# SowpatiLab/ribbit

Hardware: AMD Instinct MI355X
Metric: Gbases/s scanned (m=2..100) (higher is better)
Workload: dtype u32 bit planes

## Files before the change

### ribbit_amd/csrc/kernels.hip

```cpp
#include <hip/hip_runtime.h>

#include <algorithm>
#include <climits>
#include <type_traits>

#include "kernels.h"

namespace rb {

__device__ __forceinline__ uint32_t funnel(uint32_t hi, uint32_t lo, uint32_t sh) {
    return __builtin_amdgcn_alignbit(hi, lo, sh);
}

template <unsigned TT>
__device__ __forceinline__ uint32_t bitop3(uint32_t a, uint32_t b, uint32_t c) {
    return __builtin_amdgcn_bitop3_b32(a, b, c, TT);
}

__global__ __launch_bounds__(256) void pack_kernel(const uint8_t *__restrict__ ascii, int64_t length,
                                                   uint32_t *__restrict__ hi, uint32_t *__restrict__ lo,
                                                   uint32_t *__restrict__ brk, int64_t total_words,
                                                   uint32_t *__restrict__ zero_words, int n_zero) {
    const int64_t t = (int64_t)blockIdx.x * blockDim.x + threadIdx.x;
    if (blockIdx.x == 0)
// ... 103 lines not shown
    int cnt = 0;
#pragma unroll
    for (int k = 0; k < WORDS_PER_LANE; k++) cnt += __popc(Sv[k]) + __popc(Ev[k]);
    const int incl = wave_inclusive_scan(cnt);
    const int total = __builtin_amdgcn_readlane(incl, 63);
    if (staged + total > EV_STAGE) sink_flush(sink, stage, staged, lane);
    const bool direct = total > EV_STAGE;
    uint32_t idx = (uint32_t)(incl - cnt);
    uint64_t *gdst = nullptr;
    if (direct) {
        uint32_t base = 0;
        if (lane == 0) base = atomicAdd(&sink.counters[sink.shard * EV_COUNTER_STRIDE], (uint32_t)total);
        idx += (uint32_t)__builtin_amdgcn_readfirstlane((int)base);
        gdst = sink.events + (size_t)sink.shard * sink.region_cap;
    } else {
        idx += (uint32_t)staged;
    }
#pragma unroll
    for (int k = 0; k < WORDS_PER_LANE; k++) {
        uint32_t both = Sv[k] | Ev[k];
        while (both) {
            const uint32_t b = (uint32_t)__builtin_ctz(both);
            both &= both - 1u;
            const uint32_t pos = ((word0 + (uint32_t)k) << 5) + b;
            const uint32_t kind = ((Sv[k] >> b) & 1u) ? (uint32_t)EV_START : end_kind(k, b, pos);
            const uint64_t e = ev_pack(pos, mlen, kind);
            if (direct) { if (idx < sink.region_cap) gdst[idx] = e; }
            else stage[idx] = e;
            idx++;
        }
    }
    if (!direct) staged += total;
    __builtin_amdgcn_wave_barrier();
}

constexpr int K = WORDS_PER_LANE;

#ifndef RB_COOP_MAX_LANES
#define RB_COOP_MAX_LANES 16
#endif
constexpr int COOP_SRC = 16;
struct CoopScratch { uint32_t w[COOP_SRC][20]; };

__device__ __forceinline__ void stage_events_coop(const uint32_t (&S)[WORDS_PER_LANE], const uint32_t (&E)[WORDS_PER_LANE], uint32_t word0, uint32_t mlen,
                                                  uint32_t brk_at, const uint32_t *s_brk, uint32_t length, CoopScratch &sc, const EventSink &sink,
                                                  volatile uint64_t *stage, int &staged, int lane) {
    uint32_t Sv[WORDS_PER_LANE], Ev[WORDS_PER_LANE];
#pragma unroll
    for (int k = 0; k < WORDS_PER_LANE; k++) {
        Sv[k] = S[k]; Ev[k] = E[k];
        asm volatile("" : "+v"(Sv[k]), "+v"(Ev[k]));
    }
    int cnt = 0;
#pragma unroll
    for (int k = 0; k < WORDS_PER_LANE; k++) cnt += __popc(Sv[k] | Ev[k]);
    const int incl = wave_inclusive_scan(cnt);
    const int total = __builtin_amdgcn_readlane(incl, 63);
    if (staged + total > EV_STAGE) sink_flush(sink, stage, staged, lane);
    const bool direct = total > EV_STAGE;
    uint32_t first = (uint32_t)(incl - cnt);
    uint64_t *gdst = nullptr;
    if (direct) {
        uint32_t base = 0;
        if (lane == 0) base = atomicAdd(&sink.counters[sink.shard * EV_COUNTER_STRIDE], (uint32_t)total);
        first += (uint32_t)__builtin_amdgcn_readfirstlane((int)base);
        gdst = sink.events + (size_t)sink.shard * sink.region_cap;
    } else {
        first += (uint32_t)staged;
    }
    unsigned long long todo = __ballot(cnt != 0);
    const int r = lane >> 2, j = lane & 3;
    do {
        const int rank = (int)__builtin_amdgcn_mbcnt_hi((uint32_t)(todo >> 32), __builtin_amdgcn_mbcnt_lo((uint32_t)todo, 0u));
        const bool mine = ((todo >> lane) & 1ull) != 0ull && rank < COOP_SRC;
        if (mine) {
            uint32_t *row = sc.w[rank];
#pragma unroll
            for (int k = 0; k < WORDS_PER_LANE; k++) { row[k] = Sv[k]; row[WORDS_PER_LANE + k] = Ev[k]; }
            row[16] = word0; row[17] = mlen; row[18] = brk_at; row[19] = first;
        }
        const unsigned long long handled = __ballot(mine);
        const int nsrc = __popcll(handled);
        todo &= ~handled;
        __builtin_amdgcn_wave_barrier();
        uint32_t s0 = 0, s1 = 0, e0 = 0, e1 = 0;
        if (r < nsrc) { s0 = sc.w[r][2 * j]; s1 = sc.w[r][2 * j + 1]; e0 = sc.w[r][WORDS_PER_LANE + 2 * j]; e1 = sc.w[r][WORDS_PER_LANE + 2 * j + 1]; }
        const int c = __popc(s0 | e0) + __popc(s1 | e1);
        const int q0 = __builtin_amdgcn_update_dpp(0, c, 0x00, 0xf, 0xf, true);
        const int q1 = __builtin_amdgcn_update_dpp(0, c, 0x55, 0xf, 0xf, true);
        const int q2 = __builtin_amdgcn_update_dpp(0, c, 0xaa, 0xf, 0xf, true);
        if (c != 0) {
            const uint32_t w0 = sc.w[r][16], ml = sc.w[r][17], bb = sc.w[r][18];
            uint32_t idx = sc.w[r][19] + (uint32_t)((j > 0 ? q0 : 0) + (j > 1 ? q1 : 0) + (j > 2 ? q2 : 0));
            auto expand = [&](uint32_t sw, uint32_t ew, uint32_t k) {
                uint32_t both = sw | ew;
                while (both) {
                    const uint32_t b = (uint32_t)__builtin_ctz(both);
                    both &= both - 1u;
                    const uint32_t pos = ((w0 + k) << 5) + b;
                    uint32_t kind = (uint32_t)EV_START;
                    if (!((sw >> b) & 1u))
                        kind = pos >= length ? (uint32_t)EV_END_EOS : (((s_brk[bb + k] >> b) & 1u) ? (uint32_t)EV_END_N : (uint32_t)EV_END_ZERO);
                    const uint64_t e = ev_pack(pos, ml, kind);
                    if (direct) { if (idx < sink.region_cap) gdst[idx] = e; }
                    else stage[idx] = e;
                    idx++;
                }
            };
            expand(s0, e0, 2u * (uint32_t)j);
            expand(s1, e1, 2u * (uint32_t)j + 1u);
        }
        __builtin_amdgcn_wave_barrier();
    } while (RB_COOP_MAX_LANES > COOP_SRC && todo != 0ull);
    if (!direct) staged += total;
}
__device__ __forceinline__ void group_filter(const uint32_t (&PASS)[K + 2], const uint32_t (&EVAL)[K + 2], int tj, uint32_t (&SV)[K + 1],
                                             uint32_t (&DR)[K]) {
    uint32_t J[K + 2], W[K + 2];
#pragma unroll
    for (int j = K + 1; j >= 1; j--) J[j] = PASS[j] | funnel(PASS[j], PASS[j - 1], 31);
    J[0] = PASS[0] | (PASS[0] << 1);
#pragma unroll
    for (int j = K + 1; j >= 1; j--) J[j] = J[j] | funnel(J[j], J[j - 1], 30);
    J[0] = J[0] | (J[0] << 2);
#pragma unroll
    for (int j = K + 1; j >= 1; j--) J[j] = J[j] | funnel(J[j], J[j - 1], 28);
    J[0] = J[0] | (J[0] << 4);
#pragma unroll
    for (int j = 0; j < K + 1; j++) J[j] = J[j] & funnel(J[j + 1], J[j], 1);
    J[K + 1] = J[K + 1] & (J[K + 1] >> 1);
#pragma unroll
    for (int j = 0; j < K + 1; j++) J[j] = J[j] & funnel(J[j + 1], J[j], 2);
    J[K + 1] = J[K + 1] & (J[K + 1] >> 2);
#pragma unroll
    for (int j = 0; j < K + 1; j++) J[j] = J[j] & funnel(J[j + 1], J[j], 4);
    J[K + 1] = J[K + 1] & (J[K + 1] >> 4);
#pragma unroll
    for (int j = 0; j < K + 2; j++) J[j] |= PASS[j];
#pragma unroll
    for (int j = 0; j < K + 2; j++) W[j] = J[j];
    {
        int span = 1;
#pragma unroll
        for (int step = 0; step < 4; step++) {
            const int sh = min(span, tj - span);
            if (sh > 0) {
#pragma unroll
                for (int j = 0; j < K + 1; j++) W[j] = W[j] & funnel(W[j + 1], W[j], (uint32_t)sh);
                W[K + 1] = W[K + 1] & (W[K + 1] >> sh);
                span += sh;
            }
        }
        span = 1;
#pragma unroll
        for (int step = 0; step < 4; step++) {
            const int sh = min(span, tj - span);
            if (sh > 0) {
#pragma unroll
                for (int j = K + 1; j >= 1; j--) W[j] = W[j] | funnel(W[j], W[j - 1], (uint32_t)(32 - sh));
                W[0] = W[0] | (W[0] << sh);
                span += sh;
            }
        }
    }
    auto special_ends = [&](int j) {
        const uint32_t jprev = j > 0 ? funnel(J[j], J[j - 1], 31) : (J[0] << 1);
        const uint32_t ev8 = j < K + 1 ? funnel(EVAL[j + 1], EVAL[j], 8) : (EVAL[K + 1] >> 8);
        const uint32_t g = ~J[j] & jprev & ~(EVAL[j] & ev8);
        return j == 0 ? 0u : (j == K + 1 ? (g & 0x0000ffffu) : g);
    };
    uint32_t special = 0;
#pragma unroll
    for (int j = 1; j < K + 2; j++) special |= special_ends(j);
    if (__ballot(special != 0) != 0ull) {
        uint32_t G[K + 2], JL[K + 2];
#pragma unroll
        for (int j = 0; j < K + 2; j++) { JL[j] = J[j]; G[j] = special_ends(j); }
#pragma unroll
        for (int j = 0; j < K + 1; j++) G[j] = funnel(G[j + 1], G[j], 1) & J[j];
        G[K + 1] = (G[K + 1] >> 1) & J[K + 1];
#pragma unroll
        for (int sh = 1; sh <= 8; sh <<= 1) {
#pragma unroll
            for (int j = 0; j < K + 1; j++) G[j] |= funnel(G[j + 1], G[j], (uint32_t)sh) & JL[j];
            G[K + 1] |= (G[K + 1] >> sh) & JL[K + 1];
#pragma unroll
            for (int j = 0; j < K + 1; j++) JL[j] = JL[j] & funnel(JL[j + 1], JL[j], (uint32_t)sh);
            JL[K + 1] = JL[K + 1] & (JL[K + 1] >> sh);
        }
#pragma unroll
        for (int j = 0; j < K + 1; j++) W[j] |= G[j];
    }
#pragma unroll
    for (int j = 0; j < K + 1; j++) SV[j] = W[j];
#pragma unroll
    for (int k = 0; k < K; k++) {
        const uint32_t jprev = funnel(J[k + 1], J[k], 31);
        const uint32_t svprev = funnel(W[k + 1], W[k], 31);
        DR[k] = ~J[k + 1] & jprev & ~svprev;
    }
}

constexpr int LDS_EXTRA = 40;

template <bool UNIFORM>
__device__ __forceinline__ uint32_t perfect_edges(const uint32_t (&Z)[K + 2], uint32_t t3, uint32_t t4, uint32_t t5,
                                                  uint32_t back, uint32_t (&SQ)[K], uint32_t (&EQ)[K]) {
    uint32_t D[K + 2];
#pragma unroll
    for (int j = 0; j < K + 1; j++) D[j] = Z[j] | funnel(Z[j + 1], Z[j], 1);
    D[K + 1] = Z[K + 1] | (Z[K + 1] >> 1);
#pragma unroll
    for (int j = 0; j < K + 1; j++) D[j] = D[j] | funnel(D[j + 1], D[j], 2);
    D[K + 1] = D[K + 1] | (D[K + 1] >> 2);
#pragma unroll
    for (int j = 0; j < K + 1; j++) D[j] = D[j] | funnel(D[j + 1], D[j], t3);
    D[K + 1] = D[K + 1] | (D[K + 1] >> t3);
#pragma unroll
    for (int j = 0; j < K + 1; j++) D[j] = D[j] | funnel(D[j + 1], D[j], t4);
    if (!UNIFORM || t5) {
        D[K + 1] = D[K + 1] | (D[K + 1] >> t4);
#pragma unroll
        for (int j = 0; j < K + 1; j++) D[j] = D[j] | funnel(D[j + 1], D[j], t5);
    }
    uint32_t any = 0;
#pragma unroll
    for (int k = 0; k < K; k++) {
        const int j = k + 1;
        const uint32_t prev_z = funnel(Z[j], Z[j - 1], 31);
        const uint32_t d_back = funnel(D[j], D[j - 1], back);
        SQ[k] = prev_z & ~D[j];
        EQ[k] = Z[j] & ~d_back;
        any = bitop3<0xFE>(SQ[k], EQ[k], any);
    }
    return any;
}

constexpr int CAND_CAP = 64;
#ifndef RB_CAND_DIRECT
#define RB_CAND_DIRECT 32
#endif
constexpr int CAND_DIRECT = RB_CAND_DIRECT;
struct CandQueue {
    uint32_t z[K + 2][CAND_CAP];
    uint32_t tag[CAND_CAP];
};

#ifndef RB_PERFECT_WAVES
#define RB_PERFECT_WAVES 4
#endif
__global__ __launch_bounds__(256) __attribute__((amdgpu_waves_per_eu(RB_PERFECT_WAVES, RB_PERFECT_WAVES))) void scan_perfect_kernel(DevicePlanes pl, PerfectLaunch pp, int motifs_per_block,
                                                           uint64_t *__restrict__ events,
                                                           uint32_t *__restrict__ counters) {
    __shared__ uint32_t s_hi[TILE_WORDS + LDS_EXTRA];
    __shared__ uint32_t s_lo[TILE_WORDS + LDS_EXTRA];
    __shared__ uint32_t s_brk[TILE_WORDS + 8];
    __shared__ uint64_t s_stage[4][EV_STAGE];
    __shared__ CandQueue s_cand[4];
    __shared__ CoopScratch s_coop[4];

    const int lane = threadIdx.x & 63;
    const int wave = __builtin_amdgcn_readfirstlane((int)(threadIdx.x >> 6));
    const int64_t tile_base = (int64_t)blockIdx.x * TILE_WORDS;

    const int bm_lo = pp.m_lo + (int)blockIdx.y * motifs_per_block;
    const int bm_hi = min(pp.m_hi, bm_lo + motifs_per_block - 1);
    const int q_hi = bm_hi >> 5;

    const int n_ext = TILE_WORDS + 4 + q_hi;
    for (int i = threadIdx.x; i < n_ext; i += 256) {
        s_hi[i] = pl.hi[tile_base - 1 + i];
        s_lo[i] = pl.lo[tile_base - 1 + i];
    }
    for (int i = threadIdx.x; i < TILE_WORDS + 2; i += 256) s_brk[i] = pl.brk[tile_base - 1 + i];
    __syncthreads();

    const int wm_lo = bm_lo + wave;
    const int wm_hi = bm_hi;
    if (wm_lo > wm_hi) return;

    const int lb = lane * K;
    uint32_t H[K + 2], Lo[K + 2], Bk[K + 2];
#pragma unroll
    for (int j = 0; j < K + 2; j++) { H[j] = s_hi[lb + j]; Lo[j] = s_lo[lb + j]; Bk[j] = s_brk[lb + j]; }

    uint32_t Hq[K + 3], Lq[K + 3];
    int cur_q = -1;
    const uint32_t length = (uint32_t)pl.length;
    const uint32_t word0 = (uint32_t)(tile_base + lb);

    EventSink sink;
    sink.events = events;
    sink.counters = counters;
    sink.region_cap = pp.ev_cap / EV_SHARDS;
    sink.shard = (blockIdx.x * 4u + (uint32_t)wave + blockIdx.y) % EV_SHARDS;
    volatile uint64_t *stage = s_stage[wave];
    int staged = 0;

    CandQueue &cq = s_cand[wave];
    int queued = 0;
    auto flush_candidates = [&]() {
        if (queued == 0) return;
        const bool live = lane < queued;
        const uint32_t tag = live ? cq.tag[lane] : 0u;
        const uint32_t src = tag & 0xffu, qm = tag >> 8;
        uint32_t Zq[K + 2];
#pragma unroll
        for (int j = 0; j < K + 2; j++) Zq[j] = live ? cq.z[j][lane] : 0xffffffffu;
        const int c1 = (qm <= 6u) ? 12 - (int)qm : (int)qm;
        const int sp = live ? min(c1, 32) : 32;
        const uint32_t t3 = (uint32_t)min(4, sp - 4);
        const uint32_t t4 = (uint32_t)min(8, sp - 4 - (int)t3);
        const uint32_t t5 = (uint32_t)(sp - 4) - t3 - t4;
        uint32_t SQ[K], EQ[K];
        uint32_t any = perfect_edges<false>(Zq, t3, t4, t5, 32u - (uint32_t)sp, SQ, EQ);
        if (!live) {
            any = 0;
#pragma unroll
            for (int k = 0; k < K; k++) { SQ[k] = 0; EQ[k] = 0; }
        }
#ifdef RB_ABLATE_STAGING
        const unsigned long long with_events = __ballot(any == 0xdeadbeefu);
#else
        const unsigned long long with_events = __ballot(any != 0);
#endif
        if (with_events != 0ull) {
            const uint32_t src_word0 = (uint32_t)tile_base + src * (uint32_t)K;
            if (__popcll(with_events) <= RB_COOP_MAX_LANES)
                stage_events_coop(SQ, EQ, src_word0, qm, src * (uint32_t)K + 1u, s_brk, length, s_coop[wave], sink, stage, staged, lane);
            else
                stage_events(SQ, EQ, src_word0, qm, sink, stage, staged, lane, [&](int k, uint32_t b, uint32_t pos) {
                    if (pos >= length) return (uint32_t)EV_END_EOS;
                    return ((s_brk[src * (uint32_t)K + (uint32_t)k + 1u] >> b) & 1u) ? (uint32_t)EV_END_N : (uint32_t)EV_END_ZERO;
                });
        }
        queued = 0;
        __builtin_amdgcn_wave_barrier();
    };

    for (int m = wm_lo; m <= wm_hi; m += 4) {
        const int q = m >> 5;
        const uint32_t r = (uint32_t)m & 31u;
        if (q != cur_q) {
            cur_q = q;
#pragma unroll
            for (int j = 0; j < K + 3; j++) { Hq[j] = s_hi[lb + j + q]; Lq[j] = s_lo[lb + j + q]; }
        }
        const int c1 = (m <= 6) ? 12 - m : m;
        const int sp = min(c1, 32);
        const uint32_t t3 = (uint32_t)min(4, sp - 4);
        const uint32_t t4 = (uint32_t)min(8, sp - 4 - (int)t3);
        const uint32_t t5 = (uint32_t)(sp - 4) - t3 - t4;

        uint32_t Z[K + 2];
#pragma unroll
        for (int j = 0; j < K + 2; j++) {
            const uint32_t hs = funnel(Hq[j + 1], Hq[j], r);
            const uint32_t ls = funnel(Lq[j + 1], Lq[j], r);
            Z[j] = bitop3<0xF6>(bitop3<0xBE>(H[j], hs, Bk[j]), Lo[j], ls);
        }
        if (sp >= 7) {
            bool cand;
            if (sp >= 31) {
                typedef unsigned short half2 __attribute__((ext_vector_type(2)));
                auto pk_min = [](uint32_t a, uint32_t b) {
                    const half2 m = __builtin_elementwise_min(__builtin_bit_cast(half2, a), __builtin_bit_cast(half2, b));
                    return __builtin_bit_cast(uint32_t, m);
                };
                uint32_t lowest = Z[0];
#pragma unroll
                for (int j = 1; j < K + 2; j++) lowest = pk_min(lowest, Z[j]);
                cand = (((lowest - 0x00010001u) & ~lowest) & 0x80008000u) != 0;
            } else {
                const uint32_t ones = sp >= 15 ? 0x01010101u : 0x11111111u;
                const uint32_t tops = sp >= 15 ? 0x80808080u : 0x88888888u;
                uint32_t hit = 0;
#pragma unroll
                for (int j = 0; j < K + 2; j++) hit = bitop3<0xBA>(Z[j] - ones, Z[j], hit);
                cand = (hit & tops) != 0;
            }
#ifdef RB_ABLATE_CHAIN
            const unsigned long long mask = __ballot(cand && Z[0] == 0xdeadbeefu);
#else
            const unsigned long long mask = __ballot(cand);
#endif
            if (mask == 0ull) continue;
            const int n = __popcll(mask);
            if (n <= CAND_DIRECT) {
                if (queued + n > CAND_CAP) flush_candidates();
                if (cand) {
                    const int slot = queued + (int)__builtin_amdgcn_mbcnt_hi((uint32_t)(mask >> 32), __builtin_amdgcn_mbcnt_lo((uint32_t)mask, 0u));
#pragma unroll
                    for (int j = 0; j < K + 2; j++) cq.z[j][slot] = Z[j];
                    cq.tag[slot] = (uint32_t)lane | ((uint32_t)m << 8);
                }
                queued += n;
                __builtin_amdgcn_wave_barrier();
                continue;
            }
        }
        uint32_t SQ[K], EQ[K];
        const uint32_t any = perfect_edges<true>(Z, t3, t4, t5, 32u - (uint32_t)sp, SQ, EQ);
#ifdef RB_ABLATE_STAGING
        const unsigned long long with_events = __ballot(any == 0xdeadbeefu);
#else
        const unsigned long long with_events = __ballot(any != 0);
#endif
        if (with_events != 0ull) {
            if (__popcll(with_events) <= RB_COOP_MAX_LANES)
                stage_events_coop(SQ, EQ, word0, (uint32_t)m, (uint32_t)lb + 1u, s_brk, length, s_coop[wave], sink, stage, staged, lane);
            else
                stage_events(SQ, EQ, word0, (uint32_t)m, sink, stage, staged, lane, [&](int k, uint32_t b, uint32_t pos) {
                    if (pos >= length) return (uint32_t)EV_END_EOS;
                    return ((Bk[k + 1] >> b) & 1u) ? (uint32_t)EV_END_N : (uint32_t)EV_END_ZERO;
                });
        }
    }
    flush_candidates();
    sink_flush(sink, stage, staged, lane);
}

static ScanSplit scan_split(const PerfectLaunch &pp, int nm, int64_t want_y, int max_y) {
    int motifs_per_block;
    if (pp.motifs_per_block > 0) {
        motifs_per_block = std::min(pp.motifs_per_block, nm);
    } else {
        const int gy = (int)(want_y < 1 ? 1 : (want_y > max_y ? max_y : want_y));
        motifs_per_block = (nm + gy - 1) / gy;
    }
    ScanSplit sp;
    sp.motifs_per_block = motifs_per_block;
    sp.grid_y = (nm + motifs_per_block - 1) / motifs_per_block;
    return sp;
}

ScanSplit launch_scan_perfect(const DevicePlanes &pl, const PerfectLaunch &pp, uint64_t *events, uint32_t *counters,
                              hipStream_t stream) {
    const int nm = pp.m_hi - pp.m_lo + 1;
    if (nm <= 0 || pl.ntiles <= 0) return {};
    const ScanSplit sp = scan_split(pp, nm, (2048 + pl.ntiles - 1) / pl.ntiles, (nm + 3) / 4);
    dim3 grid((unsigned)pl.ntiles, (unsigned)sp.grid_y);
    hipLaunchKernelGGL(scan_perfect_kernel, grid, dim3(256), 0, stream, pl, pp, sp.motifs_per_block, events, counters);
    return sp;
}

template <int ALLOWED>
__global__ __launch_bounds__(256) void scan_window_kernel(DevicePlanes pl, PerfectLaunch pp, int motifs_per_block,
                                                          uint64_t *__restrict__ events,
                                                          uint32_t *__restrict__ counters) {
    __shared__ uint32_t s_hi[TILE_WORDS + LDS_EXTRA];
    __shared__ uint32_t s_lo[TILE_WORDS + LDS_EXTRA];
    __shared__ uint32_t s_brk[TILE_WORDS + 8];
    __shared__ uint64_t s_stage[4][EV_STAGE];

    const int lane = threadIdx.x & 63;
    const int wave = __builtin_amdgcn_readfirstlane((int)(threadIdx.x >> 6));
    const int64_t tile_base = (int64_t)blockIdx.x * TILE_WORDS;

    const int bm_lo = pp.m_lo + (int)blockIdx.y * motifs_per_block;
    const int bm_hi = min(pp.m_hi, bm_lo + motifs_per_block - 1);
    const int q_hi = bm_hi >> 5;
    const int n_ext = TILE_WORDS + 4 + q_hi;
    for (int i = threadIdx.x; i < n_ext; i += 256) {
        s_hi[i] = pl.hi[tile_base - 1 + i];
        s_lo[i] = pl.lo[tile_base - 1 + i];
    }
    for (int i = threadIdx.x; i < TILE_WORDS + 2; i += 256) s_brk[i] = pl.brk[tile_base - 1 + i];
    __syncthreads();

    const int wm_lo = bm_lo + wave;
    const int wm_hi = bm_hi;
    if (wm_lo > wm_hi) return;

    const int lb = lane * K;
    uint32_t H[K + 2], Lo[K + 2];
    uint32_t EVAL[K + 1];
    {
        uint32_t B[K + 2];
#pragma unroll
        for (int j = 0; j < K + 2; j++) { H[j] = s_hi[lb + j]; Lo[j] = s_lo[lb + j]; B[j] = s_brk[lb + j]; }
#pragma unroll
        for (int j = 0; j < K + 1; j++) B[j] |= funnel(B[j + 1], B[j], 1);
        B[K + 1] |= B[K + 1] >> 1;
#pragma unroll
        for (int j = 0; j < K + 1; j++) B[j] |= funnel(B[j + 1], B[j], 2);
        B[K + 1] |= B[K + 1] >> 2;
#pragma unroll
        for (int j = 0; j < K + 1; j++) EVAL[j] = ~(B[j] | funnel(B[j + 1], B[j], 4));
    }

    uint32_t Hq[K + 3], Lq[K + 3];
    int cur_q = -1;
    const uint32_t length = (uint32_t)pl.length;
    const uint32_t word0 = (uint32_t)(tile_base + lb);

    EventSink sink;
    sink.events = events;
    sink.counters = counters;
    sink.region_cap = pp.ev_cap / EV_SHARDS;
    sink.shard = (blockIdx.x * 4u + (uint32_t)wave + blockIdx.y) % EV_SHARDS;
    volatile uint64_t *stage = s_stage[wave];
    int staged = 0;

    for (int m = wm_lo; m <= wm_hi; m += 4) {
        const int q = m >> 5;
        const uint32_t r = (uint32_t)m & 31u;
        if (q != cur_q) {
            cur_q = q;
#pragma unroll
            for (int j = 0; j < K + 3; j++) { Hq[j] = s_hi[lb + j + q]; Lq[j] = s_lo[lb + j + q]; }
        }
        uint32_t A1[K + 2], B1[K + 2], C1[K + 2];
#pragma unroll
        for (int j = 0; j < K + 2; j++) {
            const uint32_t hs = funnel(Hq[j + 1], Hq[j], r);
            const uint32_t ls = funnel(Lq[j + 1], Lq[j], r);
            A1[j] = (H[j] ^ hs) | (Lo[j] ^ ls);
        }
#pragma unroll
        for (int j = 0; j < K + 2; j++) {
            const uint32_t sa = (j <= K) ? funnel(A1[j + 1 <= K + 1 ? j + 1 : j], A1[j], 1) : (A1[j] >> 1);
            B1[j] = A1[j] & sa;
            A1[j] = A1[j] | sa;
        }
#pragma unroll
        for (int j = 0; j < K + 2; j++) {
            const uint32_t sa = (j <= K) ? funnel(A1[j + 1 <= K + 1 ? j + 1 : j], A1[j], 2) : (A1[j] >> 2);
            const uint32_t sb = (j <= K) ? funnel(B1[j + 1 <= K + 1 ? j + 1 : j], B1[j], 2) : (B1[j] >> 2);
            if (ALLOWED == 2) C1[j] = (B1[j] & sa) | (A1[j] & sb);
            B1[j] = B1[j] | sb | (A1[j] & sa);
            A1[j] = A1[j] | sa;
        }
        uint32_t PASS[K + 1];
#pragma unroll
        for (int j = 0; j < K + 1; j++) {
            const uint32_t sa = funnel(A1[j + 1], A1[j], 4);
            const uint32_t sb = funnel(B1[j + 1], B1[j], 4);
            uint32_t bad;
            if (ALLOWED == 2) {
                const uint32_t sc = funnel(C1[j + 1], C1[j], 4);
                bad = C1[j] | sc | (B1[j] & sa) | (A1[j] & sb);
            } else {
                bad = B1[j] | sb | (A1[j] & sa);
            }
            PASS[j] = EVAL[j] & ~bad;
        }
        uint32_t ST[K], EN[K];
        uint32_t any = 0;
#pragma unroll
        for (int k = 0; k < K; k++) {
            const uint32_t prev = funnel(PASS[k + 1], PASS[k], 31);
            ST[k] = PASS[k + 1] & ~prev;
            EN[k] = ~PASS[k + 1] & prev;
            any |= ST[k] | EN[k];
        }
        if (__ballot(any != 0) != 0ull) {
            stage_events(ST, EN, word0, (uint32_t)m, sink, stage, staged, lane, [&](int k, uint32_t b, uint32_t pos) {
                if ((EVAL[k + 1] >> b) & 1u) return (uint32_t)EV_END_ZERO;
                return (pos + 7u >= length) ? (uint32_t)EV_END_EOS : (uint32_t)EV_END_N;
            });
        }
    }
    sink_flush(sink, stage, staged, lane);
}

ScanSplit launch_scan_window(const DevicePlanes &pl, const PerfectLaunch &pp, int allowed_mismatches, uint64_t *events,
                             uint32_t *counters, hipStream_t stream) {
    const int nm = pp.m_hi - pp.m_lo + 1;
    if (nm <= 0 || pl.ntiles <= 0) return {};
    const ScanSplit sp = scan_split(pp, nm, (2048 + pl.ntiles - 1) / pl.ntiles, (nm + 3) / 4);
    dim3 grid((unsigned)pl.ntiles, (unsigned)sp.grid_y);
    if (allowed_mismatches == 1)
        hipLaunchKernelGGL(scan_window_kernel<1>, grid, dim3(256), 0, stream, pl, pp, sp.motifs_per_block, events, counters);
    else
        hipLaunchKernelGGL(scan_window_kernel<2>, grid, dim3(256), 0, stream, pl, pp, sp.motifs_per_block, events, counters);
    return sp;
}

constexpr int RUN_SAT = 1 << 20;

__global__ __launch_bounds__(256) __attribute__((amdgpu_waves_per_eu(2, 4))) void scan_anchored_kernel(DevicePlanes pl, PerfectLaunch pp, int motifs_per_block, int hl,
                                                            uint32_t *__restrict__ xa, int64_t xa_stride) {
    __shared__ uint32_t s_hi[64 * K + LDS_EXTRA];
    __shared__ uint32_t s_lo[64 * K + LDS_EXTRA];

    const int lane = threadIdx.x & 63;
    const int wave = __builtin_amdgcn_readfirstlane((int)(threadIdx.x >> 6));
    const int64_t tile_base = (int64_t)blockIdx.x * anchored_tile_words(hl);
    const int64_t first = tile_base - (int64_t)hl * K - 1;

    const int bm_lo = pp.m_lo + (int)blockIdx.y * motifs_per_block;
    const int bm_hi = min(pp.m_hi, bm_lo + motifs_per_block - 1);
    const int q_hi = (bm_hi + 2) >> 5;
    const int n_ext = 64 * K + 4 + q_hi;
    for (int i = threadIdx.x; i < n_ext; i += 256) {
        s_hi[i] = pl.hi[first + i];
        s_lo[i] = pl.lo[first + i];
    }
    __syncthreads();

    const int nmb = bm_hi - bm_lo + 1;
    const int per = (nmb + 3) >> 2;
    const int wm_lo = bm_lo + wave * per;
    const int wm_hi = min(bm_hi, wm_lo + per - 1);
    if (wm_lo > wm_hi) return;

    const int lb = lane * K;
    const bool own_lane = lane >= hl && lane < 64 - hl;
    uint32_t H[K + 2], Lo[K + 2];
#pragma unroll
    for (int j = 0; j < K + 2; j++) { H[j] = s_hi[lb + j]; Lo[j] = s_lo[lb + j]; }

    const int64_t w_own0 = tile_base + (int64_t)(lane - hl) * K;
    const int64_t length = pl.length;
    const int64_t lane_lo = (w_own0 - 1) * 32, lane_hi = (w_own0 + K + 1) * 32;
    const bool edge_lane = lane_lo < 0 || lane_hi > length - (int64_t)(wm_hi + 2);
    const bool edge_wave = __ballot(edge_lane) != 0ull;

    uint32_t Hq[K + 3], Lq[K + 3];
    int cur_q = -1;

    uint32_t AN[5][K + 2];
#pragma unroll
    for (int a = 0; a < 5; a++)
#pragma unroll
        for (int j = 0; j < K + 2; j++) AN[a][j] = 0;

    const int s_first = max(1, wm_lo - 2);
    const int s_last = wm_hi + 2;
    auto step = [&](auto slot_c, int s) {
        constexpr int R = decltype(slot_c)::value;
        constexpr int R1 = (R + 4) % 5, R3 = (R + 2) % 5, R4 = (R + 1) % 5;
        const int q = s >> 5;
        const uint32_t r = (uint32_t)s & 31u;
        if (q != cur_q) {
            cur_q = q;
#pragma unroll
            for (int j = 0; j < K + 3; j++) { Hq[j] = s_hi[lb + j + q]; Lq[j] = s_lo[lb + j + q]; }
        }
        uint32_t X[K];
#pragma unroll
        for (int k = 0; k < K; k++) {
            const uint32_t hs = funnel(Hq[k + 2], Hq[k + 1], r);
            const uint32_t ls = funnel(Lq[k + 2], Lq[k + 1], r);
            X[k] = ~((H[k + 1] ^ hs) | (Lo[k + 1] ^ ls));
        }
        if (edge_wave) {
#pragma unroll
            for (int k = 0; k < K; k++) {
                const int64_t bp = (w_own0 + k) * 32;
                const int64_t f = (length - s) - bp;
                const uint32_t force = f <= 0 ? 0xffffffffu : (f >= 32 ? 0u : (0xffffffffu << (uint32_t)f));
                X[k] = (bp < 0) ? 0u : (X[k] | force);
            }
        }
        const int two_s = 2 * s;
        int lead1[K], trail1[K];
        int span_lead = 0, span_trail = 0;
        bool alive = true;
#pragma unroll
        for (int k = 0; k < K; k++) {
            const uint32_t nx = ~X[k];
            lead1[k] = nx ? __builtin_ctz(nx) : 32;
            trail1[k] = nx ? __builtin_clz(nx) : 32;
            span_lead += alive ? lead1[k] : 0;
            alive = alive && (nx == 0u);
        }
        const bool span_full = alive;
        alive = true;
#pragma unroll
        for (int k = K - 1; k >= 0; k--) {
            span_trail += alive ? trail1[k] : 0;
            alive = alive && (X[k] == 0xffffffffu);
        }
        int accL = span_trail, accR = span_lead, fullL = span_full ? 1 : 0, fullR = fullL;
        for (int d = 1; d < hl; d <<= 1) {
            int a2 = __shfl_up(accL, d), f2 = __shfl_up(fullL, d);
            if (lane < d) { a2 = 0; f2 = 0; }
            accL = min(accL + (fullL ? a2 : 0), RUN_SAT);
            fullL &= f2;
            a2 = __shfl_down(accR, d); f2 = __shfl_down(fullR, d);
            if (lane + d > 63) { a2 = 0; f2 = 0; }
            accR = min(accR + (fullR ? a2 : 0), RUN_SAT);
            fullR &= f2;
        }
        int left_in = __shfl_up(accL, 1);
        int right_in = __shfl_down(accR, 1);
        if (lane == 0) left_in = 0;
        if (lane == 63) right_in = 0;
        int CL[K], CR[K];
        {
            int c = left_in;
#pragma unroll
            for (int k = 0; k < K; k++) { CL[k] = c; c = (X[k] == 0xffffffffu) ? min(c + 32, RUN_SAT) : trail1[k]; }
            c = right_in;
#pragma unroll
            for (int k = K - 1; k >= 0; k--) { CR[k] = c; c = (X[k] == 0xffffffffu) ? min(c + 32, RUN_SAT) : lead1[k]; }
        }
#pragma unroll
        for (int k = 0; k < K; k++) {
            const uint32_t x = X[k];
            const bool isfull = x == 0xffffffffu;
            const uint32_t mask_low = isfull ? 0xffffffffu : ((1u << lead1[k]) - 1u);
            const uint32_t mask_high = (isfull || trail1[k] == 0) ? 0u : (0xffffffffu << (32 - trail1[k]));
            const int low_len = CL[k] + lead1[k] + (isfull ? CR[k] : 0);
            const int high_len = trail1[k] + CR[k];
            const uint32_t inter = x & ~mask_low & ~mask_high;
            const uint32_t r3 = inter & (inter >> 1) & (inter >> 2);
            uint32_t keep = r3 | (r3 << 1) | (r3 << 2);
            if (two_s <= 30) {
                uint32_t rr = inter;
                for (int span = 1; span < two_s;) { const int sh = min(span, two_s - span); rr &= rr >> sh; span += sh; }
                for (int span = 1; span < two_s;) { const int sh = min(span, two_s - span); rr |= rr << sh; span += sh; }
                keep &= ~rr;
            }
            if (lead1[k] > 0 && low_len >= 3 && low_len < two_s) keep |= mask_low;
            if (high_len >= 3 && high_len < two_s) keep |= mask_high;
            AN[R][k + 1] = keep;
        }

        const int m = s - 2;
// ... 637 lines not shown
```

Measured before the change: 432.4.

## Specialize candidate scan loop per period class with tight inner loop

Restructures the per-motif-length scan into segments by class (nibble, byte, half-word, in-place), each running a templated tight inner loop that only computes the candidate probe and ballot, and exits to the outer loop only for dense or flush work. The candidate reduction is rebalanced into pairwise trees to shorten dependency chains. The flush lambda now reads clamped slots instead of using per-lane select predicates. This aims to cut per-iteration branching and uniform recomputation in the hot loop, at the cost of more complex control flow and more code duplication.

```diff
diff --git a/ribbit_amd/csrc/kernels.hip b/ribbit_amd/csrc/kernels.hip
--- a/ribbit_amd/csrc/kernels.hip
+++ b/ribbit_amd/csrc/kernels.hip
@@ -429,13 +429,14 @@
     auto flush_candidates = [&]() {
         if (queued == 0) return;
         const bool live = lane < queued;
-        const uint32_t tag = live ? cq.tag[lane] : 0u;
+        const int slot = min(lane, queued - 1);
+        const uint32_t tag = cq.tag[slot];
         const uint32_t src = tag & 0xffu, qm = tag >> 8;
         uint32_t Zq[K + 2];
 #pragma unroll
-        for (int j = 0; j < K + 2; j++) Zq[j] = live ? cq.z[j][lane] : 0xffffffffu;
+        for (int j = 0; j < K + 2; j++) Zq[j] = cq.z[j][slot];
         const int c1 = (qm <= 6u) ? 12 - (int)qm : (int)qm;
-        const int sp = live ? min(c1, 32) : 32;
+        const int sp = min(c1, 32);
         const uint32_t t3 = (uint32_t)min(4, sp - 4);
         const uint32_t t4 = (uint32_t)min(8, sp - 4 - (int)t3);
         const uint32_t t5 = (uint32_t)(sp - 4) - t3 - t4;
@@ -465,85 +466,133 @@
         __builtin_amdgcn_wave_barrier();
     };
 
-    for (int m = wm_lo; m <= wm_hi; m += 4) {
-        const int q = m >> 5;
-        const uint32_t r = (uint32_t)m & 31u;
-        if (q != cur_q) {
-            cur_q = q;
-#pragma unroll
-            for (int j = 0; j < K + 3; j++) { Hq[j] = s_hi[lb + j + q]; Lq[j] = s_lo[lb + j + q]; }
-        }
-        const int c1 = (m <= 6) ? 12 - m : m;
-        const int sp = min(c1, 32);
-        const uint32_t t3 = (uint32_t)min(4, sp - 4);
-        const uint32_t t4 = (uint32_t)min(8, sp - 4 - (int)t3);
-        const uint32_t t5 = (uint32_t)(sp - 4) - t3 - t4;
-
-        uint32_t Z[K + 2];
-#pragma unroll
-        for (int j = 0; j < K + 2; j++) {
-            const uint32_t hs = funnel(Hq[j + 1], Hq[j], r);
-            const uint32_t ls = funnel(Lq[j + 1], Lq[j], r);
-            Z[j] = bitop3<0xF6>(bitop3<0xBE>(H[j], hs, Bk[j]), Lo[j], ls);
-        }
-        if (sp >= 7) {
-            bool cand;
-            if (sp >= 31) {
-                typedef unsigned short half2 __attribute__((ext_vector_type(2)));
-                auto pk_min = [](uint32_t a, uint32_t b) {
-                    const half2 m = __builtin_elementwise_min(__builtin_bit_cast(half2, a), __builtin_bit_cast(half2, b));
-                    return __builtin_bit_cast(uint32_t, m);
-                };
-                uint32_t lowest = Z[0];
-#pragma unroll
-                for (int j = 1; j < K + 2; j++) lowest = pk_min(lowest, Z[j]);
-                cand = (((lowest - 0x00010001u) & ~lowest) & 0x80008000u) != 0;
+    enum : int { CLS_INPLACE, CLS_NIBBLE, CLS_BYTE, CLS_HALF };
+    enum : int { ACT_FINAL, ACT_PARK, ACT_DENSE };
+    int m = wm_lo, seg_hi = 0;
+    uint32_t Z[K + 2];
+    unsigned long long mask = 0ull;
+
+    auto park = [&](bool cand, int n) {
+        if (cand) {
+            const int slot = queued + (int)__builtin_amdgcn_mbcnt_hi((uint32_t)(mask >> 32), __builtin_amdgcn_mbcnt_lo((uint32_t)mask, 0u));
+#pragma unroll
+            for (int j = 0; j < K + 2; j++) cq.z[j][slot] = Z[j];
+            cq.tag[slot] = (uint32_t)lane | ((uint32_t)m << 8);
+        }
+        queued += n;
+        __builtin_amdgcn_wave_barrier();
+    };
+
+    auto fast_loop = [&](auto cls) -> bool {
+        constexpr int CLS = decltype(cls)::value;
+        uint32_t probe = 0, tops = 0;
+        for (;;) {
+          do {
+            const uint32_t r = (uint32_t)m & 31u;
+#pragma unroll
+            for (int j = 0; j < K + 2; j++) {
+                const uint32_t hs = funnel(Hq[j + 1], Hq[j], r);
+                const uint32_t ls = funnel(Lq[j + 1], Lq[j], r);
+                Z[j] = bitop3<0xF6>(bitop3<0xBE>(H[j], hs, Bk[j]), Lo[j], ls);
+            }
+            if constexpr (CLS == CLS_INPLACE) {
+                mask = ~0ull;
+                return true;
             } else {
-                const uint32_t ones = sp >= 15 ? 0x01010101u : 0x11111111u;
-                const uint32_t tops = sp >= 15 ? 0x80808080u : 0x88888888u;
-                uint32_t hit = 0;
-#pragma unroll
-                for (int j = 0; j < K + 2; j++) hit = bitop3<0xBA>(Z[j] - ones, Z[j], hit);
-                cand = (hit & tops) != 0;
+                if constexpr (CLS == CLS_HALF) {
+                    typedef unsigned short half2 __attribute__((ext_vector_type(2)));
+                    auto pk_min = [](uint32_t a, uint32_t b) {
+                        const half2 lo2 = __builtin_elementwise_min(__builtin_bit_cast(half2, a), __builtin_bit_cast(half2, b));
+                        return __builtin_bit_cast(uint32_t, lo2);
+                    };
+                    uint32_t p[(K + 2) / 2];
+#pragma unroll
+                    for (int j = 0; j < (K + 2) / 2; j++) p[j] = pk_min(Z[2 * j], Z[2 * j + 1]);
+                    const uint32_t lowest = pk_min(pk_min(pk_min(p[0], p[1]), pk_min(p[2], p[3])), p[4]);
+                    probe = (lowest - 0x00010001u) & ~lowest;
+                    tops = 0x80008000u;
+                } else {
+                    constexpr uint32_t ones = CLS == CLS_BYTE ? 0x01010101u : 0x11111111u;
+                    tops = CLS == CLS_BYTE ? 0x80808080u : 0x88888888u;
+                    uint32_t p[(K + 2) / 2];
+#pragma unroll
+                    for (int j = 0; j < (K + 2) / 2; j++)
+                        p[j] = bitop3<0xBA>(Z[2 * j + 1] - ones, Z[2 * j + 1], bitop3<0x30>(Z[2 * j] - ones, Z[2 * j], 0u));
+                    probe = bitop3<0xFE>(bitop3<0xFE>(p[0], p[1], p[2]), p[3], p[4]);
+                }
+                static_assert((K + 2) / 2 == 5, "the reductions above are written for ten words");
+                const bool cand = (probe & tops) != 0;
+#ifdef RB_ABLATE_CHAIN
+                mask = __ballot(cand && Z[0] == 0xdeadbeefu);
+#else
+                mask = __ballot(cand);
+#endif
             }
-#ifdef RB_ABLATE_CHAIN
-            const unsigned long long mask = __ballot(cand && Z[0] == 0xdeadbeefu);
+          } while (mask == 0ull && (m += 4) <= seg_hi);
+          asm volatile("" : "+s"(mask));
+          if (mask == 0ull) return false;
+          const int n = __popcll(mask);
+          if (n > CAND_DIRECT || queued + n > CAND_CAP) return true;
+          park((probe & tops) != 0, n);
+          if ((m += 4) > seg_hi) return false;
+        }
+    };
+
+    for (;;) {
+        int act = ACT_FINAL;
+        if (m <= wm_hi) {
+            const int q = m >> 5;
+            if (q != cur_q) {
+                cur_q = q;
+#pragma unroll
+                for (int j = 0; j < K + 3; j++) { Hq[j] = s_hi[lb + j + q]; Lq[j] = s_lo[lb + j + q]; }
+            }
+            bool left;
+            if (m >= 31) {
+                seg_hi = min(wm_hi, m | 31);
+                left = fast_loop(std::integral_constant<int, CLS_HALF>());
+            } else if (m >= 15) {
+                seg_hi = min(wm_hi, 30);
+                left = fast_loop(std::integral_constant<int, CLS_BYTE>());
+            } else if (m != 6) {
+                seg_hi = min(wm_hi, m < 6 ? 5 : 14);
+                left = fast_loop(std::integral_constant<int, CLS_NIBBLE>());
+            } else {
+                seg_hi = 6;
+                left = fast_loop(std::integral_constant<int, CLS_INPLACE>());
+            }
+            if (!left) continue;
+            act = (m == 6 || __popcll(mask) > CAND_DIRECT) ? ACT_DENSE : ACT_PARK;
+        }
+        if (act == ACT_DENSE) {
+            const int c1 = (m <= 6) ? 12 - m : m;
+            const int sp = min(c1, 32);
+            const uint32_t t3 = (uint32_t)min(4, sp - 4);
+            const uint32_t t4 = (uint32_t)min(8, sp - 4 - (int)t3);
+            const uint32_t t5 = (uint32_t)(sp - 4) - t3 - t4;
+            uint32_t SQ[K], EQ[K];
+            const uint32_t any = perfect_edges<true>(Z, t3, t4, t5, 32u - (uint32_t)sp, SQ, EQ);
+#ifdef RB_ABLATE_STAGING
+            const unsigned long long with_events = __ballot(any == 0xdeadbeefu);
 #else
-            const unsigned long long mask = __ballot(cand);
+            const unsigned long long with_events = __ballot(any != 0);
 #endif
-            if (mask == 0ull) continue;
-            const int n = __popcll(mask);
-            if (n <= CAND_DIRECT) {
-                if (queued + n > CAND_CAP) flush_candidates();
-                if (cand) {
-                    const int slot = queued + (int)__builtin_amdgcn_mbcnt_hi((uint32_t)(mask >> 32), __builtin_amdgcn_mbcnt_lo((uint32_t)mask, 0u));
-#pragma unroll
-                    for (int j = 0; j < K + 2; j++) cq.z[j][slot] = Z[j];
-                    cq.tag[slot] = (uint32_t)lane | ((uint32_t)m << 8);
-                }
-                queued += n;
-                __builtin_amdgcn_wave_barrier();
-                continue;
+            if (with_events != 0ull) {
+                if (__popcll(with_events) <= RB_COOP_MAX_LANES)
+                    stage_events_coop(SQ, EQ, word0, (uint32_t)m, (uint32_t)lb + 1u, s_brk, length, s_coop[wave], sink, stage, staged, lane);
+                else
+                    stage_events(SQ, EQ, word0, (uint32_t)m, sink, stage, staged, lane, [&](int k, uint32_t b, uint32_t pos) {
+                        if (pos >= length) return (uint32_t)EV_END_EOS;
+                        return ((Bk[k + 1] >> b) & 1u) ? (uint32_t)EV_END_N : (uint32_t)EV_END_ZERO;
+                    });
             }
-        }
-        uint32_t SQ[K], EQ[K];
-        const uint32_t any = perfect_edges<true>(Z, t3, t4, t5, 32u - (uint32_t)sp, SQ, EQ);
-#ifdef RB_ABLATE_STAGING
-        const unsigned long long with_events = __ballot(any == 0xdeadbeefu);
-#else
-        const unsigned long long with_events = __ballot(any != 0);
-#endif
-        if (with_events != 0ull) {
-            if (__popcll(with_events) <= RB_COOP_MAX_LANES)
-                stage_events_coop(SQ, EQ, word0, (uint32_t)m, (uint32_t)lb + 1u, s_brk, length, s_coop[wave], sink, stage, staged, lane);
-            else
-                stage_events(SQ, EQ, word0, (uint32_t)m, sink, stage, staged, lane, [&](int k, uint32_t b, uint32_t pos) {
-                    if (pos >= length) return (uint32_t)EV_END_EOS;
-                    return ((Bk[k + 1] >> b) & 1u) ? (uint32_t)EV_END_N : (uint32_t)EV_END_ZERO;
-                });
-        }
-    }
-    flush_candidates();
+        } else {
+            flush_candidates();
+            if (act == ACT_FINAL) break;
+            park(((mask >> lane) & 1ull) != 0ull, __popcll(mask));
+        }
+        m += 4;
+    }
     sink_flush(sink, stage, staged, lane);
 }
 
```

Result: slower. 426.7 (-1.3%).
